# Sue1347/SMSUT-MedicalImgSegmentation

Measured on AMD Instinct MI355X. Metric: slices/sec uganConsisTrainer step @256x256, higher is better.
Workload: dtype f32

## Files before the change

### smsut-medicalimgsegmentation_amd/csrc/conv1x1.hip

```cpp
#include "common.h"

namespace {

typedef float f32x4 __attribute__((ext_vector_type(4)));
constexpr int TPB = 256;

__device__ __forceinline__ f32x4 mfma16(float a, float b, f32x4 c) {
  return __builtin_amdgcn_mfma_f32_16x16x4f32(a, b, c, 0, 0, 0);
}

template <int MR, int NR, bool DUAL = false, bool PS = false>
__global__ void __launch_bounds__(TPB)
conv1x1_fwd(const float* __restrict__ x, const float* __restrict__ w, float* __restrict__ y, float* __restrict__ stats,
            int64_t P, int HW, int Kdim, int Ndim, int transposed, float* __restrict__ y2 = nullptr, int split = 0,
            const float* __restrict__ x2 = nullptr, int ca = 0, int ps_w = 0) {
  constexpr int CO_T = 16 * NR;
  extern __shared__ float w_s[];
  const int tid = threadIdx.x, lane = tid & 63, wave = tid >> 6;
  const int lm = lane & 15, kq = lane >> 4;
  const int co0 = blockIdx.y * CO_T;
  const int chunks = (Kdim + 15) / 16;
  for (int u = tid; u < chunks * 4 * CO_T; u += TPB) {
    const int n = u % CO_T;
    const int kg = (u / CO_T) * 4;
    const int ng = co0 + n;
    float4 v = make_float4(0.f, 0.f, 0.f, 0.f);
    if (ng < Ndim && kg < Kdim) {
      if constexpr (PS) {
        const int cout = Ndim >> 2, tap = ng / cout;
        const float* p = w + ((size_t)tap * Kdim + kg) * cout + (ng - tap * cout);
        v.x = p[0]; v.y = p[cout]; v.z = p[2 * (size_t)cout]; v.w = p[3 * (size_t)cout];
      } else if (!transposed) {
        const float* p = w + (size_t)kg * Ndim + ng;
        v.x = p[0]; v.y = p[Ndim]; v.z = p[2 * (size_t)Ndim]; v.w = p[3 * (size_t)Ndim];
      } else {
        v = *(const float4*)(w + (size_t)ng * Kdim + kg);
      }
    }
    *(float4*)(w_s + (size_t)u * 4) = v;
  }
  __syncthreads();

  const int64_t p0 = ((int64_t)blockIdx.x * 4 + wave) * (16 * MR);
  if (p0 >= P) return;
  f32x4 acc[MR][NR];
#pragma unroll
  for (int i = 0; i < MR; ++i)
#pragma unroll
    for (int j = 0; j < NR; ++j) acc[i][j] = (f32x4){0.f, 0.f, 0.f, 0.f};
  const float* xp[MR];
  const float* xq[MR];
  bool pok[MR];
  const int sa = DUAL ? ca : Kdim;
#pragma unroll
  for (int i = 0; i < MR; ++i) {
    const int64_t p = p0 + i * 16 + lm;
    pok[i] = p < P;
    xp[i] = x + (size_t)(pok[i] ? p : 0) * sa + 4 * kq;
    xq[i] = DUAL ? x2 + (size_t)(pok[i] ? p : 0) * (Kdim - ca) + 4 * kq - ca : xp[i];
  }
  for (int c = 0; c < chunks; ++c) {
    const bool kok = c * 16 + 4 * kq < Kdim;
    const bool second = DUAL && c * 16 >= ca;
    f32x4 a[MR], b[NR];
#pragma unroll
    for (int i = 0; i < MR; ++i)
      a[i] = (pok[i] && kok) ? *(const f32x4*)((second ? xq[i] : xp[i]) + c * 16) : (f32x4){0.f, 0.f, 0.f, 0.f};
#pragma unroll
    for (int j = 0; j < NR; ++j) b[j] = *(const f32x4*)(w_s + ((size_t)(c * 4 + kq) * CO_T + j * 16 + lm) * 4);
#pragma unroll
    for (int s = 0; s < 4; ++s)
#pragma unroll
      for (int i = 0; i < MR; ++i)
#pragma unroll
        for (int j = 0; j < NR; ++j) acc[i][j] = mfma16(a[i][s], b[j][s], acc[i][j]);
  }
#pragma unroll
  for (int j = 0; j < NR; ++j) {
    const int co = co0 + j * 16 + lm;
    const bool hi = y2 && co0 + j * 16 >= split;
    float* const yo = hi ? y2 : y;
    const int os = !y2 ? Ndim : (hi ? Ndim - split : split);
    const int oc = hi ? co - split : co;
    float s1 = 0.f, s2 = 0.f;
    if constexpr (PS) {
      const int cout = Ndim >> 2, tap = (co0 + j * 16) / cout, cc = co - tap * cout;
      const int W2 = 2 * ps_w;
#pragma unroll
      for (int i = 0; i < MR; ++i)
#pragma unroll
        for (int r = 0; r < 4; ++r) {
          const int64_t p = p0 + i * 16 + 4 * kq + r;
          if (p < P && co < Ndim) {
            const int row = (int)p / ps_w;
            const int wx = (int)p - row * ps_w;
            y[((size_t)(2 * row + (tap >> 1)) * W2 + 2 * wx + (tap & 1)) * cout + cc] = acc[i][j][r];
          }
        }
      continue;
    }
#pragma unroll
    for (int i = 0; i < MR; ++i)
#pragma unroll
      for (int r = 0; r < 4; ++r) {
        const int64_t p = p0 + i * 16 + 4 * kq + r;
        if (p < P && co < Ndim) {
          const float v = acc[i][j][r];
          yo[(size_t)p * os + oc] = v;
          s1 += v; s2 += v * v;
        }
      }
    if (stats) {
      s1 += __shfl_xor(s1, 16, 64); s2 += __shfl_xor(s2, 16, 64);
      s1 += __shfl_xor(s1, 32, 64); s2 += __shfl_xor(s2, 32, 64);
      if (kq == 0 && co < Ndim) {
        const int tiles = HW / (16 * MR);
        const int64_t n_img = p0 / HW;
        const int tile = (int)((p0 % HW) / (16 * MR));
        float* o = stats + (((size_t)n_img * tiles + tile) * Ndim + co) * 2;
        o[0] = s1; o[1] = s2;
      }
    }
  }
}

#ifndef W1_UNR
#define W1_UNR 4
#endif
template <int CIT, int COT, bool PS = false>
__global__ void __launch_bounds__(TPB)
conv1x1_wgrad(const float* __restrict__ x, const float* __restrict__ gy, float* __restrict__ part, int64_t P, int Cin,
              int Cout, int64_t pix_per_split, const float* __restrict__ x2 = nullptr, int ca = 0, int ps_w = 0) {
  __shared__ float red[CIT * COT * 64 * 4];
  const int tid = threadIdx.x, lane = tid & 63, wave = tid >> 6;
  const int lm = lane & 15, kq = lane >> 4;
  const int ci0 = blockIdx.y * (16 * CIT), co0 = blockIdx.z * (16 * COT);
  const int64_t pb = (int64_t)blockIdx.x * pix_per_split;
  const int64_t pe = min(pb + pix_per_split, P);
  f32x4 acc[CIT][COT];
#pragma unroll
  for (int i = 0; i < CIT; ++i)
#pragma unroll
    for (int j = 0; j < COT; ++j) acc[i][j] = (f32x4){0.f, 0.f, 0.f, 0.f};
  bool iok[CIT], jok[COT];
#pragma unroll
  for (int i = 0; i < CIT; ++i) iok[i] = ci0 + i * 16 + lm < Cin;
#pragma unroll
  for (int j = 0; j < COT; ++j) jok[j] = co0 + j * 16 + lm < Cout;
  CatSrc xs[CIT];
#pragma unroll
  for (int i = 0; i < CIT; ++i) xs[i] = cat_src(x, x2, Cin, ca, ci0 + i * 16);
  const float* gb = gy + co0 + lm;
  [[maybe_unused]] const int cout = Cout >> 2;
  [[maybe_unused]] int ps_tap[COT], ps_cc[COT];
  if constexpr (PS) {
#pragma unroll
    for (int j = 0; j < COT; ++j) { ps_tap[j] = (co0 + j * 16) / cout; ps_cc[j] = co0 + j * 16 - ps_tap[j] * cout + lm; }
  }
  constexpr int UNR = W1_UNR;
  for (int64_t p0 = pb + 4 * wave + kq; p0 - kq < pe; p0 += 16 * UNR) {
    float a[UNR][CIT], b[UNR][COT];
#pragma unroll
    for (int u = 0; u < UNR; ++u) {
      const int64_t p = p0 + 16 * u;
      const bool ok = p < pe;
#pragma unroll
      for (int i = 0; i < CIT; ++i) a[u][i] = (ok && iok[i]) ? xs[i].p[(size_t)p * xs[i].stride + ci0 + i * 16 + lm - xs[i].coff] : 0.f;
      if constexpr (PS) {
        const int row = (int)p / ps_w;
        const int wx = (int)p - row * ps_w;
#pragma unroll
        for (int j = 0; j < COT; ++j)
          b[u][j] = (ok && jok[j]) ? gy[((size_t)(2 * row + (ps_tap[j] >> 1)) * (2 * ps_w) + 2 * wx + (ps_tap[j] & 1)) * cout + ps_cc[j]] : 0.f;
      } else {
#pragma unroll
        for (int j = 0; j < COT; ++j) b[u][j] = (ok && jok[j]) ? gb[(size_t)p * Cout + j * 16] : 0.f;
      }
    }
#pragma unroll
    for (int u = 0; u < UNR; ++u)
#pragma unroll
      for (int i = 0; i < CIT; ++i)
#pragma unroll
        for (int j = 0; j < COT; ++j) acc[i][j] = mfma16(a[u][i], b[u][j], acc[i][j]);
  }
  for (int src = 1; src < 4; ++src) {
    __syncthreads();
    if (wave == src) {
#pragma unroll
      for (int i = 0; i < CIT; ++i)
#pragma unroll
        for (int j = 0; j < COT; ++j) *(f32x4*)(red + ((size_t)(i * COT + j) * 64 + lane) * 4) = acc[i][j];
    }
    __syncthreads();
    if (wave == 0) {
#pragma unroll
      for (int i = 0; i < CIT; ++i)
#pragma unroll
        for (int j = 0; j < COT; ++j) acc[i][j] += *(const f32x4*)(red + ((size_t)(i * COT + j) * 64 + lane) * 4);
    }
  }
  if (wave == 0) {
    float* out = part + (size_t)blockIdx.x * Cin * Cout;
#pragma unroll
    for (int i = 0; i < CIT; ++i)
#pragma unroll
      for (int j = 0; j < COT; ++j) {
        const int co = co0 + j * 16 + lm;
#pragma unroll
        for (int r = 0; r < 4; ++r) {
          const int ci = ci0 + i * 16 + 4 * kq + r;
          if constexpr (PS) {
            if (ci < Cin && co < Cout) out[((size_t)ps_tap[j] * Cin + ci) * cout + ps_cc[j]] = acc[i][j][r];
          } else if (ci < Cin && co < Cout) out[(size_t)ci * Cout + co] = acc[i][j][r];
        }
      }
  }
}

__global__ void __launch_bounds__(TPB)
sum_parts(const float* __restrict__ part, float* __restrict__ out, int wsize, int splits) {
  __shared__ float4 sm[TPB];
  const int col = threadIdx.x & 15, sl = threadIdx.x >> 4;
  const int e = (blockIdx.x * 16 + col) * 4;
  float4 t0 = make_float4(0.f, 0.f, 0.f, 0.f), t1 = t0, t2 = t0, t3 = t0;
  if (e < wsize) {
    int c = sl;
    for (; c + 48 < splits; c += 64) {
      const float4 v0 = *(const float4*)(part + (size_t)c * wsize + e);
      const float4 v1 = *(const float4*)(part + (size_t)(c + 16) * wsize + e);
      const float4 v2 = *(const float4*)(part + (size_t)(c + 32) * wsize + e);
      const float4 v3 = *(const float4*)(part + (size_t)(c + 48) * wsize + e);
      t0.x += v0.x; t0.y += v0.y; t0.z += v0.z; t0.w += v0.w; t1.x += v1.x; t1.y += v1.y; t1.z += v1.z; t1.w += v1.w;
      t2.x += v2.x; t2.y += v2.y; t2.z += v2.z; t2.w += v2.w; t3.x += v3.x; t3.y += v3.y; t3.z += v3.z; t3.w += v3.w;
    }
    for (; c < splits; c += 16) {
      const float4 v = *(const float4*)(part + (size_t)c * wsize + e);
      t0.x += v.x; t0.y += v.y; t0.z += v.z; t0.w += v.w;
    }
  }
  sm[threadIdx.x] = make_float4((t0.x + t1.x) + (t2.x + t3.x), (t0.y + t1.y) + (t2.y + t3.y), (t0.z + t1.z) + (t2.z + t3.z),
                                (t0.w + t1.w) + (t2.w + t3.w));
  __syncthreads();
  if (sl == 0 && e < wsize) {
    float4 t = sm[col];
    for (int l = 1; l < 16; ++l) { const float4 v = sm[l * 16 + col]; t.x += v.x; t.y += v.y; t.z += v.z; t.w += v.w; }
    *(float4*)(out + e) = t;
  }
}

struct Plan1 { int splits; int64_t pps; };
inline Plan1 plan_wgrad1(int64_t P, int Cin, int Cout, int cit, int cot) {
  const int slabs = ((Cin + 16 * cit - 1) / (16 * cit)) * ((Cout + 16 * cot - 1) / (16 * cot));
  int64_t want = (1024 + slabs - 1) / slabs;
  const int64_t maxs = P / 256 > 0 ? P / 256 : 1;
  if (want > maxs) want = maxs;
  if (want < 1) want = 1;
  Plan1 p;
  p.pps = ((P + want - 1) / want + 15) / 16 * 16;
  p.splits = (int)((P + p.pps - 1) / p.pps);
  return p;
}


constexpr int THIN_MAX = 8;

template <int CI>
__global__ void __launch_bounds__(TPB)
thin1x1_dgrad(const float* __restrict__ gy, const float* __restrict__ w, float* __restrict__ gx, int64_t P, int CO) {
  constexpr int Q = CI / 4;
  __shared__ float wt[THIN_MAX * CI];
  for (int u = threadIdx.x; u < THIN_MAX * CI; u += TPB) {
    const int k = u / CI, ci = u % CI;
    wt[u] = k < CO ? w[ci * CO + k] : 0.f;
  }
  __syncthreads();
  const int64_t total = P * Q;
  for (int64_t i = (int64_t)blockIdx.x * TPB + threadIdx.x; i < total; i += (int64_t)gridDim.x * TPB) {
    const int c4 = (int)(i % Q);
    const int64_t px = i / Q;
    float g[THIN_MAX];
#pragma unroll
    for (int k = 0; k < THIN_MAX; ++k) g[k] = k < CO ? gy[px * CO + k] : 0.f;
    f32x4 o = {0.f, 0.f, 0.f, 0.f};
#pragma unroll
    for (int k = 0; k < THIN_MAX; ++k) o += g[k] * *(const f32x4*)(wt + k * CI + c4 * 4);
    *(f32x4*)(gx + i * 4) = o;
  }
}

template <int CI>
__global__ void __launch_bounds__(TPB)
thin1x1_wgrad(const float* __restrict__ x, const float* __restrict__ gy, float* __restrict__ part, int64_t P, int CO) {
  constexpr int Q = CI / 4;
  static_assert(Q <= 64 && (Q & (Q - 1)) == 0, "lanes sharing a channel group sit Q apart inside a wave");
  __shared__ float sm[4 * Q * 4 * THIN_MAX];
  f32x4 acc[THIN_MAX];
#pragma unroll
  for (int k = 0; k < THIN_MAX; ++k) acc[k] = (f32x4){0.f, 0.f, 0.f, 0.f};
  const int64_t total = P * Q;
  const int64_t stride = (int64_t)gridDim.x * TPB;
  auto step = [&](int64_t i) {
    const int64_t px = i / Q;
    const f32x4 xv = *(const f32x4*)(x + i * 4);
#pragma unroll
    for (int k = 0; k < THIN_MAX; ++k) {
      const float g = k < CO ? gy[px * CO + k] : 0.f;
      acc[k] += g * xv;
    }
  };
  int64_t i = (int64_t)blockIdx.x * TPB + threadIdx.x;
  for (; i + stride < total; i += 2 * stride) { step(i); step(i + stride); }
  for (; i < total; i += stride) step(i);
  for (int off = Q; off < 64; off <<= 1) {
#pragma unroll
    for (int k = 0; k < THIN_MAX; ++k)
#pragma unroll
      for (int j = 0; j < 4; ++j) acc[k][j] += __shfl_xor(acc[k][j], off, 64);
  }
  const int lane = threadIdx.x & 63, wv = threadIdx.x >> 6;
  if (lane < Q) {
#pragma unroll
    for (int k = 0; k < THIN_MAX; ++k) *(f32x4*)(sm + ((wv * Q + lane) * THIN_MAX + k) * 4) = acc[k];
  }
  __syncthreads();
  if (threadIdx.x < Q) {
    const int c4 = threadIdx.x;
#pragma unroll
    for (int k = 0; k < THIN_MAX; ++k) {
      f32x4 t = *(const f32x4*)(sm + ((0 * Q + c4) * THIN_MAX + k) * 4);
#pragma unroll
      for (int w4 = 1; w4 < 4; ++w4) t += *(const f32x4*)(sm + ((w4 * Q + c4) * THIN_MAX + k) * 4);
#pragma unroll
      for (int j = 0; j < 4; ++j) part[((size_t)blockIdx.x * CI + c4 * 4 + j) * THIN_MAX + k] = t[j];
    }
  }
}

__global__ void __launch_bounds__(TPB)
thin1x1_wsum(const float* __restrict__ part, float* __restrict__ gw, int blocks, int CI, int CO) {
  const int lane = threadIdx.x & 63;
  const int col = blockIdx.x * 4 + (threadIdx.x >> 6);
  if (col >= CI * THIN_MAX / 4) return;
  f32x4 t = {0.f, 0.f, 0.f, 0.f};
  for (int b = lane; b < blocks; b += 64) t += *(const f32x4*)(part + ((size_t)b * CI * THIN_MAX) + col * 4);
  for (int off = 1; off < 64; off <<= 1)
#pragma unroll
    for (int j = 0; j < 4; ++j) t[j] += __shfl_xor(t[j], off, 64);
  if (lane == 0) {
    const int ci = col / 2, k0 = (col & 1) * 4;
#pragma unroll
    for (int j = 0; j < 4; ++j)
      if (k0 + j < CO) gw[ci * CO + k0 + j] = t[j];
  }
}

constexpr int THIN_WGRAD_BLOCKS = 1024;

}

extern "C" {

int smsut_conv1x1_supported(int Kdim, int Ndim) { return Kdim >= 4 && (Kdim % 4) == 0 && Kdim <= 512 && Ndim >= 1; }

int smsut_conv1x1_tiles(int N, int HW, int Ndim) {
  const int64_t P = (int64_t)N * HW;
  const int mr = (P / 256 >= 512) ? 4 : 1;
  (void)Ndim;
  return (HW % (16 * mr) == 0) ? HW / (16 * mr) : 0;
}

static int conv1x1_fwd_launch(const float* x, const float* w, float* y, float* stats, int N, int HW, int Kdim, int Ndim,
                              int transposed, void* stream, float* y2, int split, const float* x2 = nullptr, int ca = 0) {
  SMSUT_REQUIRE(x && w && y && N > 0 && HW > 0 && smsut_conv1x1_supported(Kdim, Ndim));
  SMSUT_REQUIRE(!y2 || (!stats && split > 0 && split < Ndim && split % 16 == 0));
  SMSUT_REQUIRE(!x2 || (!transposed && ca > 0 && ca < Kdim && ca % 16 == 0 && (Kdim - ca) % 4 == 0));
  const int64_t P = (int64_t)N * HW;
  const int mr = (P / 256 >= 512) ? 4 : 1;
  SMSUT_REQUIRE(!stats || HW % (16 * mr) == 0);
  const int nr = Ndim <= 16 ? 1 : 2;
  const int chunks = (Kdim + 15) / 16;
  const size_t sh = (size_t)chunks * 4 * 16 * nr * 4 * sizeof(float);
  dim3 grid((unsigned)cdiv64(P, 64 * mr), (Ndim + 16 * nr - 1) / (16 * nr));
  hipStream_t st = (hipStream_t)stream;
#define LAUNCH1X1(M, R)                                                                                                      \
  do {                                                                                                                       \
    if (x2) conv1x1_fwd<M, R, true><<<grid, TPB, sh, st>>>(x, w, y, stats, P, HW, Kdim, Ndim, transposed, y2, split, x2, ca); \
    else conv1x1_fwd<M, R, false><<<grid, TPB, sh, st>>>(x, w, y, stats, P, HW, Kdim, Ndim, transposed, y2, split, nullptr, 0); \
  } while (0)
  if (mr == 4 && nr == 2) LAUNCH1X1(4, 2);
  else if (mr == 4) LAUNCH1X1(4, 1);
  else if (nr == 2) LAUNCH1X1(1, 2);
  else LAUNCH1X1(1, 1);
#undef LAUNCH1X1
  SMSUT_LAUNCH_CHECK();
  return SMSUT_OK;
}

int smsut_conv1x1_fwd(const float* x, const float* w, float* y, float* stats, int N, int HW, int Kdim, int Ndim,
                      int transposed, void* stream) {
  return conv1x1_fwd_launch(x, w, y, stats, N, HW, Kdim, Ndim, transposed, stream, nullptr, 0);
}

int smsut_conv1x1_fwd_cat(const float* xa, const float* xb, int ca, const float* w, float* y, float* stats, int N, int HW,
                          int Kdim, int Ndim, void* stream) {
  SMSUT_REQUIRE(xb);
  return conv1x1_fwd_launch(xa, w, y, stats, N, HW, Kdim, Ndim, 0, stream, nullptr, 0, xb, ca);
}

int smsut_conv1x1_fwd_split(const float* x, const float* w, float* ya, float* yb, int split, int N, int HW, int Kdim,
                            int Ndim, int transposed, void* stream) {
  SMSUT_REQUIRE(yb);
  return conv1x1_fwd_launch(x, w, ya, nullptr, N, HW, Kdim, Ndim, transposed, stream, yb, split);
}

int smsut_convT2x2_ps_supported(int Cin, int Cout) {
  return Cout == 16 && Cin <= 256 && smsut_conv1x1_supported(Cin, 4 * Cout);
}

int smsut_convT2x2_fwd_ps(const float* x, const float* w, float* y, int N, int H, int W, int Cin, int Cout, void* stream) {
  SMSUT_REQUIRE(x && w && y && N > 0 && H > 0 && W > 0 && smsut_convT2x2_ps_supported(Cin, Cout));
  const int64_t P = (int64_t)N * H * W;
  SMSUT_REQUIRE(P * 4 * Cout < (1ll << 31));
  const int Nd = 4 * Cout;
  const int mr = (P / 256 >= 512) ? 4 : 1;
  const int nr = (Nd % 64 == 0) ? 4 : 2;
  const int chunks = (Cin + 15) / 16;
  const size_t sh = (size_t)chunks * 4 * 16 * nr * 4 * sizeof(float);
  dim3 grid((unsigned)cdiv64(P, 64 * mr), Nd / (16 * nr));
  hipStream_t st = (hipStream_t)stream;
#define PS_GO(M, R) conv1x1_fwd<M, R, false, true><<<grid, TPB, sh, st>>>(x, w, y, nullptr, P, H * W, Cin, Nd, 0, nullptr, 0, nullptr, 0, W)
  if (mr == 4 && nr == 4) PS_GO(4, 4);
  else if (mr == 4) PS_GO(4, 2);
  else if (nr == 4) PS_GO(1, 4);
  else PS_GO(1, 2);
#undef PS_GO
  SMSUT_LAUNCH_CHECK();
  return SMSUT_OK;
}

int64_t smsut_convT2x2_wgrad_ps_ws(int N, int H, int W, int Cin, int Cout) {
  const int cit = Cin > 16 ? 2 : 1;
  return (int64_t)plan_wgrad1((int64_t)N * H * W, Cin, 4 * Cout, cit, 2).splits * Cin * 4 * Cout;
}

int smsut_convT2x2_wgrad_ps(const float* x, const float* gy, float* gw, float* workspace, int N, int H, int W, int Cin,
                            int Cout, void* stream) {
  SMSUT_REQUIRE(x && gy && gw && workspace && N > 0 && H > 0 && W > 0 && smsut_convT2x2_ps_supported(Cin, Cout));
  const int64_t P = (int64_t)N * H * W;
  SMSUT_REQUIRE(P * 4 * Cout < (1ll << 31));
  const int Nd = 4 * Cout;
  const int cit = Cin > 16 ? 2 : 1;
  const Plan1 p = plan_wgrad1(P, Cin, Nd, cit, 2);
  dim3 grid(p.splits, (Cin + 16 * cit - 1) / (16 * cit), Nd / 32);
  hipStream_t st = (hipStream_t)stream;
  if (cit == 2) conv1x1_wgrad<2, 2, true><<<grid, TPB, 0, st>>>(x, gy, workspace, P, Cin, Nd, p.pps, nullptr, 0, W);
  else conv1x1_wgrad<1, 2, true><<<grid, TPB, 0, st>>>(x, gy, workspace, P, Cin, Nd, p.pps, nullptr, 0, W);
  const int wsize = Cin * Nd;
  sum_parts<<<(wsize + 63) / 64, TPB, 0, st>>>(workspace, gw, wsize, p.splits);
  SMSUT_LAUNCH_CHECK();
  return SMSUT_OK;
}

int64_t smsut_conv1x1_wgrad_ws(int N, int HW, int Cin, int Cout) {
  const int cit = Cin > 16 ? 2 : 1, cot = Cout > 16 ? 2 : 1;
  return (int64_t)plan_wgrad1((int64_t)N * HW, Cin, Cout, cit, cot).splits * Cin * Cout;
}

static int conv1x1_wgrad_launch(const float* x, const float* gy, float* gw, float* workspace, int N, int HW, int Cin,
                                int Cout, void* stream, const float* x2, int ca) {
  SMSUT_REQUIRE(x && gy && gw && workspace && N > 0 && HW > 0 && Cin > 0 && Cout > 0);
  SMSUT_REQUIRE(!x2 || (ca > 0 && ca < Cin && ca % 16 == 0));
  SMSUT_REQUIRE(((int64_t)Cin * Cout) % 4 == 0);
  const int64_t P = (int64_t)N * HW;
  const int cit = Cin > 16 ? 2 : 1, cot = Cout > 16 ? 2 : 1;
  const Plan1 p = plan_wgrad1(P, Cin, Cout, cit, cot);
  dim3 grid(p.splits, (Cin + 16 * cit - 1) / (16 * cit), (Cout + 16 * cot - 1) / (16 * cot));
  hipStream_t st = (hipStream_t)stream;
  if (cit == 2 && cot == 2) conv1x1_wgrad<2, 2><<<grid, TPB, 0, st>>>(x, gy, workspace, P, Cin, Cout, p.pps, x2, ca);
  else if (cit == 2) conv1x1_wgrad<2, 1><<<grid, TPB, 0, st>>>(x, gy, workspace, P, Cin, Cout, p.pps, x2, ca);
  else if (cot == 2) conv1x1_wgrad<1, 2><<<grid, TPB, 0, st>>>(x, gy, workspace, P, Cin, Cout, p.pps, x2, ca);
  else conv1x1_wgrad<1, 1><<<grid, TPB, 0, st>>>(x, gy, workspace, P, Cin, Cout, p.pps, x2, ca);
  const int wsize = Cin * Cout;
  sum_parts<<<(wsize + 63) / 64, TPB, 0, st>>>(workspace, gw, wsize, p.splits);
  SMSUT_LAUNCH_CHECK();
  return SMSUT_OK;
}

int smsut_conv1x1_wgrad(const float* x, const float* gy, float* gw, float* workspace, int N, int HW, int Cin, int Cout,
                        void* stream) {
  return conv1x1_wgrad_launch(x, gy, gw, workspace, N, HW, Cin, Cout, stream, nullptr, 0);
}

int smsut_conv1x1_wgrad_cat(const float* xa, const float* xb, int ca, const float* gy, float* gw, float* workspace, int N,
                            int HW, int Cin, int Cout, void* stream) {
  SMSUT_REQUIRE(xb);
  return conv1x1_wgrad_launch(xa, gy, gw, workspace, N, HW, Cin, Cout, stream, xb, ca);
}

int smsut_conv1x1_thin_supported(int Cin, int Cout) {
  return (Cin == 8 || Cin == 16 || Cin == 32 || Cin == 64) && Cout >= 1 && Cout <= THIN_MAX;
}

int smsut_conv1x1_thin_dgrad(const float* gy, const float* w, float* gx, int N, int HW, int Cin, int Cout, void* stream) {
  SMSUT_REQUIRE(gy && w && gx && N > 0 && HW > 0 && smsut_conv1x1_thin_supported(Cin, Cout));
  const int64_t P = (int64_t)N * HW;
  hipStream_t st = (hipStream_t)stream;
  const int grid = ew_grid(P * (Cin / 4));
  switch (Cin) {
    case 8: thin1x1_dgrad<8><<<grid, TPB, 0, st>>>(gy, w, gx, P, Cout); break;
    case 16: thin1x1_dgrad<16><<<grid, TPB, 0, st>>>(gy, w, gx, P, Cout); break;
    case 32: thin1x1_dgrad<32><<<grid, TPB, 0, st>>>(gy, w, gx, P, Cout); break;
    default: thin1x1_dgrad<64><<<grid, TPB, 0, st>>>(gy, w, gx, P, Cout); break;
  }
  SMSUT_LAUNCH_CHECK();
  return SMSUT_OK;
}

int64_t smsut_conv1x1_thin_wgrad_ws(int Cin) { return (int64_t)THIN_WGRAD_BLOCKS * Cin * THIN_MAX; }

int smsut_conv1x1_thin_wgrad(const float* x, const float* gy, float* gw, float* workspace, int N, int HW, int Cin,
                             int Cout, void* stream) {
  SMSUT_REQUIRE(x && gy && gw && workspace && N > 0 && HW > 0 && smsut_conv1x1_thin_supported(Cin, Cout));
  const int64_t P = (int64_t)N * HW;
  hipStream_t st = (hipStream_t)stream;
  int blocks = (int)cdiv64(P * (Cin / 4), 2 * TPB);
  if (blocks > THIN_WGRAD_BLOCKS) blocks = THIN_WGRAD_BLOCKS;
  switch (Cin) {
    case 8: thin1x1_wgrad<8><<<blocks, TPB, 0, st>>>(x, gy, workspace, P, Cout); break;
    case 16: thin1x1_wgrad<16><<<blocks, TPB, 0, st>>>(x, gy, workspace, P, Cout); break;
    case 32: thin1x1_wgrad<32><<<blocks, TPB, 0, st>>>(x, gy, workspace, P, Cout); break;
    default: thin1x1_wgrad<64><<<blocks, TPB, 0, st>>>(x, gy, workspace, P, Cout); break;
  }
  thin1x1_wsum<<<(Cin * THIN_MAX / 4 + 3) / 4, TPB, 0, st>>>(workspace, gw, blocks, Cin, Cout);
  SMSUT_LAUNCH_CHECK();
  return SMSUT_OK;
}

}
```

Measured before the change: 828.3.

## Persist conv1x1 forward waves over multiple pixel tiles and vectorize weight/output access

The forward 1x1 conv kernel now lets each wave loop over T consecutive pixel tiles, so the weight slab staged in LDS is reused and fewer blocks are launched. It swaps the MFMA operand order so each lane holds four consecutive output channels and can write results with one 16-byte store. It loads weights into LDS with float4 reads and an in-register transpose, and computes BN stats through a per-wave LDS transpose scratch. It also adds a waves-per-EU occupancy hint and a non-vector fallback for unaligned pointers. The costs are more template variants, extra LDS for the stats path, and possible imbalance when T>1.

```diff
diff --git a/smsut-medicalimgsegmentation_amd/csrc/conv1x1.hip b/smsut-medicalimgsegmentation_amd/csrc/conv1x1.hip
--- a/smsut-medicalimgsegmentation_amd/csrc/conv1x1.hip
+++ b/smsut-medicalimgsegmentation_amd/csrc/conv1x1.hip
@@ -9,116 +9,185 @@
   return __builtin_amdgcn_mfma_f32_16x16x4f32(a, b, c, 0, 0, 0);
 }
 
-template <int MR, int NR, bool DUAL = false, bool PS = false>
-__global__ void __launch_bounds__(TPB)
+__host__ __device__ __forceinline__ bool aligned16(const void* p) { return ((uintptr_t)p & 15) == 0; }
+
+constexpr int TR_LD = 20;
+constexpr int TR_WAVE = 16 * TR_LD;
+
+template <int MR, int NR, bool DUAL = false, bool PS = false, bool VEC = true>
+__global__ void __launch_bounds__(TPB) __attribute__((amdgpu_waves_per_eu(MR * NR <= 4 ? 8 : 4)))
 conv1x1_fwd(const float* __restrict__ x, const float* __restrict__ w, float* __restrict__ y, float* __restrict__ stats,
-            int64_t P, int HW, int Kdim, int Ndim, int transposed, float* __restrict__ y2 = nullptr, int split = 0,
+            int64_t P, int HW, int Kdim, int Ndim, int transposed, int T, float* __restrict__ y2 = nullptr, int split = 0,
             const float* __restrict__ x2 = nullptr, int ca = 0, int ps_w = 0) {
   constexpr int CO_T = 16 * NR;
   extern __shared__ float w_s[];
-  const int tid = threadIdx.x, lane = tid & 63, wave = tid >> 6;
+  const int tid = threadIdx.x, lane = tid & 63;
+  const int wave = __builtin_amdgcn_readfirstlane(tid >> 6);
   const int lm = lane & 15, kq = lane >> 4;
   const int co0 = blockIdx.y * CO_T;
   const int chunks = (Kdim + 15) / 16;
-  for (int u = tid; u < chunks * 4 * CO_T; u += TPB) {
-    const int n = u % CO_T;
-    const int kg = (u / CO_T) * 4;
-    const int ng = co0 + n;
-    float4 v = make_float4(0.f, 0.f, 0.f, 0.f);
-    if (ng < Ndim && kg < Kdim) {
-      if constexpr (PS) {
-        const int cout = Ndim >> 2, tap = ng / cout;
-        const float* p = w + ((size_t)tap * Kdim + kg) * cout + (ng - tap * cout);
-        v.x = p[0]; v.y = p[cout]; v.z = p[2 * (size_t)cout]; v.w = p[3 * (size_t)cout];
-      } else if (!transposed) {
-        const float* p = w + (size_t)kg * Ndim + ng;
-        v.x = p[0]; v.y = p[Ndim]; v.z = p[2 * (size_t)Ndim]; v.w = p[3 * (size_t)Ndim];
-      } else {
-        v = *(const float4*)(w + (size_t)ng * Kdim + kg);
-      }
-    }
-    *(float4*)(w_s + (size_t)u * 4) = v;
-  }
-  __syncthreads();
-
-  const int64_t p0 = ((int64_t)blockIdx.x * 4 + wave) * (16 * MR);
-  if (p0 >= P) return;
-  f32x4 acc[MR][NR];
-#pragma unroll
-  for (int i = 0; i < MR; ++i)
-#pragma unroll
-    for (int j = 0; j < NR; ++j) acc[i][j] = (f32x4){0.f, 0.f, 0.f, 0.f};
-  const float* xp[MR];
-  const float* xq[MR];
-  bool pok[MR];
+  const int64_t steps = (P + 16 * MR - 1) / (16 * MR);
+  const int64_t s0 = ((int64_t)blockIdx.x * 4 + wave) * T;
+  const int nT = (int)(steps - s0 < T ? steps - s0 : T);
   const int sa = DUAL ? ca : Kdim;
-#pragma unroll
-  for (int i = 0; i < MR; ++i) {
-    const int64_t p = p0 + i * 16 + lm;
-    pok[i] = p < P;
-    xp[i] = x + (size_t)(pok[i] ? p : 0) * sa + 4 * kq;
-    xq[i] = DUAL ? x2 + (size_t)(pok[i] ? p : 0) * (Kdim - ca) + 4 * kq - ca : xp[i];
-  }
-  for (int c = 0; c < chunks; ++c) {
+  const float* xb;
+  const float* xb2;
+  unsigned rel[MR];
+  auto rows = [&](int64_t p0) {
+    xb = x + (size_t)p0 * sa;
+    xb2 = DUAL ? x2 + (size_t)p0 * (Kdim - ca) - ca : xb;
+#pragma unroll
+    for (int i = 0; i < MR; ++i) rel[i] = p0 + i * 16 + lm < P ? i * 16 + lm : 0;
+  };
+  auto fetch = [&](int c, f32x4 (&a)[MR]) {
     const bool kok = c * 16 + 4 * kq < Kdim;
     const bool second = DUAL && c * 16 >= ca;
-    f32x4 a[MR], b[NR];
+    const float* const base = second ? xb2 : xb;
+    const unsigned ld = second ? Kdim - ca : sa;
+    const unsigned koff = kok ? c * 16 + 4 * kq : (second ? ca : 0);
+#pragma unroll
+    for (int i = 0; i < MR; ++i) {
+      const f32x4 v = *(const f32x4*)(base + (rel[i] * ld + koff));
+      a[i] = kok ? v : (f32x4){0.f, 0.f, 0.f, 0.f};
+    }
+  };
+
+  if (VEC && (PS || !transposed)) {
+    constexpr int NQ = CO_T / 4;
+    for (int u = tid; u < chunks * 4 * NQ; u += TPB) {
+      const int n4 = u % NQ, kg4 = u / NQ;
+      const int kg = kg4 * 4, ng = co0 + 4 * n4;
+      float4 r0 = make_float4(0.f, 0.f, 0.f, 0.f), r1 = r0, r2 = r0, r3 = r0;
+      if (ng < Ndim && kg < Kdim) {
+        const float* p;
+        size_t ld;
+        if constexpr (PS) {
+          const int cout = Ndim >> 2, tap = ng / cout;
+          p = w + ((size_t)tap * Kdim + kg) * cout + (ng - tap * cout);
+          ld = cout;
+        } else {
+          p = w + (size_t)kg * Ndim + ng;
+          ld = Ndim;
+        }
+        r0 = *(const float4*)p; r1 = *(const float4*)(p + ld); r2 = *(const float4*)(p + 2 * ld); r3 = *(const float4*)(p + 3 * ld);
+      }
+      float* d = w_s + ((size_t)kg4 * CO_T + 4 * n4) * 4;
+      *(float4*)(d) = make_float4(r0.x, r1.x, r2.x, r3.x);
+      *(float4*)(d + 4) = make_float4(r0.y, r1.y, r2.y, r3.y);
+      *(float4*)(d + 8) = make_float4(r0.z, r1.z, r2.z, r3.z);
+      *(float4*)(d + 12) = make_float4(r0.w, r1.w, r2.w, r3.w);
+    }
+  } else {
+    for (int u = tid; u < chunks * 4 * CO_T; u += TPB) {
+      const int n = u % CO_T;
+      const int kg = (u / CO_T) * 4;
+      const int ng = co0 + n;
+      float4 v = make_float4(0.f, 0.f, 0.f, 0.f);
+      if (ng < Ndim && kg < Kdim) {
+        if constexpr (PS) {
+          const int cout = Ndim >> 2, tap = ng / cout;
+          const float* p = w + ((size_t)tap * Kdim + kg) * cout + (ng - tap * cout);
+          v.x = p[0]; v.y = p[cout]; v.z = p[2 * (size_t)cout]; v.w = p[3 * (size_t)cout];
+        } else if (!transposed) {
+          const float* p = w + (size_t)kg * Ndim + ng;
+          v.x = p[0]; v.y = p[Ndim]; v.z = p[2 * (size_t)Ndim]; v.w = p[3 * (size_t)Ndim];
+        } else {
+          v = *(const float4*)(w + (size_t)ng * Kdim + kg);
+        }
+      }
+      *(float4*)(w_s + (size_t)u * 4) = v;
+    }
+  }
+  __syncthreads();
+
+  float* const tr = w_s + (size_t)chunks * 4 * CO_T * 4 + wave * TR_WAVE;
+  for (int t = 0; t < nT; ++t) {
+    const int64_t p0 = (s0 + t) * (16 * MR);
+    f32x4 acc[MR][NR];
 #pragma unroll
     for (int i = 0; i < MR; ++i)
-      a[i] = (pok[i] && kok) ? *(const f32x4*)((second ? xq[i] : xp[i]) + c * 16) : (f32x4){0.f, 0.f, 0.f, 0.f};
-#pragma unroll
-    for (int j = 0; j < NR; ++j) b[j] = *(const f32x4*)(w_s + ((size_t)(c * 4 + kq) * CO_T + j * 16 + lm) * 4);
-#pragma unroll
-    for (int s = 0; s < 4; ++s)
-#pragma unroll
-      for (int i = 0; i < MR; ++i)
-#pragma unroll
-        for (int j = 0; j < NR; ++j) acc[i][j] = mfma16(a[i][s], b[j][s], acc[i][j]);
-  }
-#pragma unroll
-  for (int j = 0; j < NR; ++j) {
-    const int co = co0 + j * 16 + lm;
-    const bool hi = y2 && co0 + j * 16 >= split;
-    float* const yo = hi ? y2 : y;
-    const int os = !y2 ? Ndim : (hi ? Ndim - split : split);
-    const int oc = hi ? co - split : co;
-    float s1 = 0.f, s2 = 0.f;
-    if constexpr (PS) {
-      const int cout = Ndim >> 2, tap = (co0 + j * 16) / cout, cc = co - tap * cout;
-      const int W2 = 2 * ps_w;
-#pragma unroll
-      for (int i = 0; i < MR; ++i)
-#pragma unroll
-        for (int r = 0; r < 4; ++r) {
-          const int64_t p = p0 + i * 16 + 4 * kq + r;
-          if (p < P && co < Ndim) {
+#pragma unroll
+      for (int j = 0; j < NR; ++j) acc[i][j] = (f32x4){0.f, 0.f, 0.f, 0.f};
+    rows(p0);
+    for (int c = 0; c < chunks; ++c) {
+      f32x4 a[MR], b[NR];
+      fetch(c, a);
+#pragma unroll
+      for (int j = 0; j < NR; ++j) b[j] = *(const f32x4*)(w_s + ((size_t)(c * 4 + kq) * CO_T + j * 16 + lm) * 4);
+#pragma unroll
+      for (int s = 0; s < 4; ++s)
+#pragma unroll
+        for (int i = 0; i < MR; ++i)
+#pragma unroll
+          for (int j = 0; j < NR; ++j) acc[i][j] = mfma16(b[j][s], a[i][s], acc[i][j]);
+    }
+#pragma unroll
+    for (int j = 0; j < NR; ++j) {
+      const int cq = co0 + j * 16 + 4 * kq;
+      if constexpr (PS) {
+        const int cout = Ndim >> 2, tap = (co0 + j * 16) / cout, cc = cq - tap * cout;
+        const int W2 = 2 * ps_w;
+#pragma unroll
+        for (int i = 0; i < MR; ++i) {
+          const int64_t p = p0 + i * 16 + lm;
+          if (p < P && cq < Ndim) {
             const int row = (int)p / ps_w;
             const int wx = (int)p - row * ps_w;
-            y[((size_t)(2 * row + (tap >> 1)) * W2 + 2 * wx + (tap & 1)) * cout + cc] = acc[i][j][r];
+            float* o = y + ((size_t)(2 * row + (tap >> 1)) * W2 + 2 * wx + (tap & 1)) * cout + cc;
+            if constexpr (VEC) {
+              *(f32x4*)o = acc[i][j];
+            } else {
+#pragma unroll
+              for (int r = 0; r < 4; ++r) o[r] = acc[i][j][r];
+            }
           }
         }
-      continue;
-    }
-#pragma unroll
-    for (int i = 0; i < MR; ++i)
-#pragma unroll
-      for (int r = 0; r < 4; ++r) {
-        const int64_t p = p0 + i * 16 + 4 * kq + r;
-        if (p < P && co < Ndim) {
-          const float v = acc[i][j][r];
-          yo[(size_t)p * os + oc] = v;
-          s1 += v; s2 += v * v;
+        continue;
+      }
+      const bool hi = y2 && co0 + j * 16 >= split;
+      float* const yo = hi ? y2 : y;
+      const int os = !y2 ? Ndim : (hi ? Ndim - split : split);
+      const int oc = hi ? cq - split : cq;
+      float* const ob = yo + (size_t)p0 * os;
+#pragma unroll
+      for (int i = 0; i < MR; ++i) {
+        const int64_t p = p0 + i * 16 + lm;
+        float* o = ob + ((unsigned)(i * 16 + lm) * (unsigned)os + (unsigned)oc);
+        if constexpr (VEC) {
+          if (p < P && cq < Ndim) *(f32x4*)o = acc[i][j];
+        } else {
+#pragma unroll
+          for (int r = 0; r < 4; ++r)
+            if (p < P && cq + r < Ndim) o[r] = acc[i][j][r];
         }
       }
-    if (stats) {
-      s1 += __shfl_xor(s1, 16, 64); s2 += __shfl_xor(s2, 16, 64);
-      s1 += __shfl_xor(s1, 32, 64); s2 += __shfl_xor(s2, 32, 64);
-      if (kq == 0 && co < Ndim) {
-        const int tiles = HW / (16 * MR);
-        const int64_t n_img = p0 / HW;
-        const int tile = (int)((p0 % HW) / (16 * MR));
-        float* o = stats + (((size_t)n_img * tiles + tile) * Ndim + co) * 2;
-        o[0] = s1; o[1] = s2;
+      if (stats) {
+#pragma clang fp contract(off)
+        const int co = co0 + j * 16 + lm;
+        float s1 = 0.f, s2 = 0.f;
+#pragma unroll
+        for (int i = 0; i < MR; ++i) {
+          __builtin_amdgcn_fence(__ATOMIC_ACQ_REL, "wavefront");
+          __builtin_amdgcn_wave_barrier();
+          *(f32x4*)(tr + lm * TR_LD + 4 * kq) = acc[i][j];
+          __builtin_amdgcn_fence(__ATOMIC_ACQ_REL, "wavefront");
+          __builtin_amdgcn_wave_barrier();
+#pragma unroll
+          for (int r = 0; r < 4; ++r) {
+            const float v = tr[(4 * kq + r) * TR_LD + lm];
+            const float vv = v * v;
+            s1 = s1 + v; s2 = s2 + vv;
+          }
+        }
+        s1 += __shfl_xor(s1, 16, 64); s2 += __shfl_xor(s2, 16, 64);
+        s1 += __shfl_xor(s1, 32, 64); s2 += __shfl_xor(s2, 32, 64);
+        if (kq == 0 && co < Ndim) {
+          const int tiles = HW / (16 * MR);
+          const int64_t n_img = p0 / HW;
+          const int tile = (int)((p0 % HW) / (16 * MR));
+          float* o = stats + (((size_t)n_img * tiles + tile) * Ndim + co) * 2;
+          o[0] = s1; o[1] = s2;
+        }
       }
     }
   }
@@ -249,6 +318,15 @@
   }
 }
 
+constexpr int C1_FULL = 2048;
+constexpr int C1_T_MAX = 8;
+inline int run_steps1(int64_t P, int mr, int slabs) {
+  const int64_t steps = cdiv64(P, 16 * mr);
+  int T = 1;
+  while (mr == 1 && T < C1_T_MAX && cdiv64(steps, 8 * T) * slabs >= C1_FULL) T *= 2;
+  return T;
+}
+
 struct Plan1 { int splits; int64_t pps; };
 inline Plan1 plan_wgrad1(int64_t P, int Cin, int Cout, int cit, int cot) {
   const int slabs = ((Cin + 16 * cit - 1) / (16 * cit)) * ((Cout + 16 * cot - 1) / (16 * cot));
@@ -378,21 +456,31 @@
   const int64_t P = (int64_t)N * HW;
   const int mr = (P / 256 >= 512) ? 4 : 1;
   SMSUT_REQUIRE(!stats || HW % (16 * mr) == 0);
-  const int nr = Ndim <= 16 ? 1 : 2;
   const int chunks = (Kdim + 15) / 16;
-  const size_t sh = (size_t)chunks * 4 * 16 * nr * 4 * sizeof(float);
-  dim3 grid((unsigned)cdiv64(P, 64 * mr), (Ndim + 16 * nr - 1) / (16 * nr));
+  const size_t scratch = stats ? 4 * TR_WAVE * sizeof(float) : 0;
+  auto image = [&](int r) { return (size_t)chunks * 4 * 16 * r * 4 * sizeof(float) + scratch; };
+  constexpr size_t LDS_MAX = 64 * 1024;
+  const int nr = Ndim <= 16 || image(2) > LDS_MAX ? 1 : 2;
+  const size_t sh = image(nr);
+  const int slabs = (Ndim + 16 * nr - 1) / (16 * nr);
+  const int T = run_steps1(P, mr, slabs);
+  dim3 grid((unsigned)cdiv64(P, 64 * mr * T), slabs);
   hipStream_t st = (hipStream_t)stream;
-#define LAUNCH1X1(M, R)                                                                                                      \
-  do {                                                                                                                       \
-    if (x2) conv1x1_fwd<M, R, true><<<grid, TPB, sh, st>>>(x, w, y, stats, P, HW, Kdim, Ndim, transposed, y2, split, x2, ca); \
-    else conv1x1_fwd<M, R, false><<<grid, TPB, sh, st>>>(x, w, y, stats, P, HW, Kdim, Ndim, transposed, y2, split, nullptr, 0); \
+  const bool vec = Ndim % 4 == 0 && aligned16(w) && aligned16(y) && aligned16(y2);
+#define GO1X1(M, R, D, V) conv1x1_fwd<M, R, D, false, V><<<grid, TPB, sh, st>>>(x, w, y, stats, P, HW, Kdim, Ndim, transposed, T, y2, split, x2, ca)
+#define LAUNCH1X1(M, R)                     \
+  do {                                      \
+    if (x2 && vec) GO1X1(M, R, true, true); \
+    else if (x2) GO1X1(M, R, true, false);  \
+    else if (vec) GO1X1(M, R, false, true); \
+    else GO1X1(M, R, false, false);         \
   } while (0)
   if (mr == 4 && nr == 2) LAUNCH1X1(4, 2);
   else if (mr == 4) LAUNCH1X1(4, 1);
   else if (nr == 2) LAUNCH1X1(1, 2);
   else LAUNCH1X1(1, 1);
 #undef LAUNCH1X1
+#undef GO1X1
   SMSUT_LAUNCH_CHECK();
   return SMSUT_OK;
 }
@@ -427,9 +515,15 @@
   const int nr = (Nd % 64 == 0) ? 4 : 2;
   const int chunks = (Cin + 15) / 16;
   const size_t sh = (size_t)chunks * 4 * 16 * nr * 4 * sizeof(float);
-  dim3 grid((unsigned)cdiv64(P, 64 * mr), Nd / (16 * nr));
+  const int T = run_steps1(P, mr, Nd / (16 * nr));
+  dim3 grid((unsigned)cdiv64(P, 64 * mr * T), Nd / (16 * nr));
   hipStream_t st = (hipStream_t)stream;
-#define PS_GO(M, R) conv1x1_fwd<M, R, false, true><<<grid, TPB, sh, st>>>(x, w, y, nullptr, P, H * W, Cin, Nd, 0, nullptr, 0, nullptr, 0, W)
+  const bool vec = aligned16(w) && aligned16(y);
+#define PS_GO(M, R)                                                                                                                  \
+  do {                                                                                                                               \
+    if (vec) conv1x1_fwd<M, R, false, true, true><<<grid, TPB, sh, st>>>(x, w, y, nullptr, P, H * W, Cin, Nd, 0, T, nullptr, 0, nullptr, 0, W); \
+    else conv1x1_fwd<M, R, false, true, false><<<grid, TPB, sh, st>>>(x, w, y, nullptr, P, H * W, Cin, Nd, 0, T, nullptr, 0, nullptr, 0, W);    \
+  } while (0)
   if (mr == 4 && nr == 4) PS_GO(4, 4);
   else if (mr == 4) PS_GO(4, 2);
   else if (nr == 4) PS_GO(1, 4);
```

After: 828.0. No clear change (-0.0%).
